# datastax/jvector

Measured on AMD Instinct MI355X. Metric: QPS@recall10>=0.95 (10Mx768); distances/sec as % HBM roofline, higher is better.
Workload: dtype f32

## Files before the change

jvector_amd/csrc/k_gsearch_ubr.hip:

```cpp
#include "jv_device.h"
#include "jv_internal.h"

#define GS_WAVE_SCOPE_BARRIER 1
#define GS_UNIFORM_SHFL 1
#include "gs_wave_hip.h"

#include "gs_body.h"

namespace jv {

static_assert(VSF_L2 == 0 && VSF_DOT == 1 && VSF_COS == 2, "gs_body.h hard-codes the kernel vsf numbering");

template <int VSF, int CH16, bool PROF>
__global__ __launch_bounds__(64) __attribute__((amdgpu_waves_per_eu(2, 2))) void graph_search_ubr_kernel(GsParams p)
{
    extern __shared__ __attribute__((aligned(16))) char gs_lds[];
    gs_worker<VSF, CH16, true, PROF, false, false, true>(p, (int)blockIdx.x, gs_lds);
}

template <int VSF, int CH16, bool PROF>
__global__ __launch_bounds__(64) __attribute__((amdgpu_waves_per_eu(2, 2))) void graph_search_ubrc_kernel(GsParams p)
{
    extern __shared__ __attribute__((aligned(16))) char gs_lds[];
    gs_worker<VSF, CH16, false, PROF, false, true, true>(p, (int)blockIdx.x, gs_lds);
}

constexpr int UBR_QB = 8;

__device__ __forceinline__ int32_t ubr_sortable(float f)
{
    const int32_t b = __builtin_bit_cast(int32_t, f);
    return b ^ ((b >> 31) & 0x7fffffff);
}
__device__ __forceinline__ float ubr_unsortable(int32_t s) { return __builtin_bit_cast(float, s ^ ((s >> 31) & 0x7fffffff)); }

__device__ __forceinline__ void ubr_wave_minmax(float &a, float &b)
{
#define JV_MM_STEP(CTRL)                                      \
    "v_min_f32_dpp %0, %0, %0 " CTRL "\n"                     \
    "v_max_f32_dpp %1, %1, %1 " CTRL "\n"                     \
    "s_nop 0\n"
    asm volatile("s_nop 1\n" JV_MM_STEP("row_shr:1 row_mask:0xf bank_mask:0xf") JV_MM_STEP("row_shr:2 row_mask:0xf bank_mask:0xf")
                     JV_MM_STEP("row_shr:4 row_mask:0xf bank_mask:0xf") JV_MM_STEP("row_shr:8 row_mask:0xf bank_mask:0xf")
                         JV_MM_STEP("row_bcast:15 row_mask:0xa bank_mask:0xf") JV_MM_STEP("row_bcast:31 row_mask:0xc bank_mask:0xf")
                 : "+v"(a), "+v"(b));
#undef JV_MM_STEP
}

template <int VSF>
__global__ __launch_bounds__(256) void ubr_table_kernel(const float *__restrict__ codebooks, const float *__restrict__ cq, int Q, int M,
                                                        uint32_t *__restrict__ tab, float *__restrict__ meta)
{
    extern __shared__ __attribute__((aligned(16))) char ubr_lds[];
    const int D = 8 * M;
    float *qs = reinterpret_cast<float *>(ubr_lds);
    float *lo = qs + UBR_QB * D;
    float *hi = lo + UBR_QB * M;
    float *qS = hi + UBR_QB * M;
    int *qbad = reinterpret_cast<int *>(qS + UBR_QB);
    const int tid = (int)threadIdx.x, lane = tid & 63, wave = tid >> 6;
    const int q0 = (int)blockIdx.x * UBR_QB;
    const int nq = min(UBR_QB, Q - q0);
    for (int i = tid; i < UBR_QB * D / 4; i += 256) {
        const int j = i / (D / 4);
        gs_f4 v = {0.0f, 0.0f, 0.0f, 0.0f};
        if (j < nq) v = reinterpret_cast<const gs_f4 *>(cq + (int64_t)(q0 + j) * D)[i - j * (D / 4)];
        reinterpret_cast<gs_f4 *>(qs)[i] = v;
    }
    if (tid < UBR_QB) qbad[tid] = 0;
    __syncthreads();
    const int H = M / 2, per_wave = H / 4;
    float lo_acc[UBR_QB], hi_acc[UBR_QB];
    uint32_t amax[UBR_QB];
#pragma unroll
    for (int j = 0; j < UBR_QB; ++j) {
        lo_acc[j] = 0.0f;
        hi_acc[j] = 0.0f;
        amax[j] = 0u;
    }
    for (int rr = 0; rr < per_wave; ++rr) {
        const int r = wave * per_wave + rr;
#pragma unroll
        for (int half = 0; half < 2; ++half) {
            const int m = r + half * H;
            gs_f4 c0[4], c1[4];
#pragma unroll
            for (int k = 0; k < 4; ++k) {
                const gs_f4 *cp = reinterpret_cast<const gs_f4 *>(codebooks + ((int64_t)m * 256 + lane + 64 * k) * 8);
                c0[k] = cp[0];
                c1[k] = cp[1];
            }
            const int slot = 2 * rr + half;
#pragma unroll
            for (int j = 0; j < UBR_QB; ++j) {
                const float *q = qs + j * D + m * 8;
                float e4[4];
#pragma unroll
                for (int k = 0; k < 4; ++k) e4[k] = gs_lut_entry_pk<VSF>(c0[k], c1[k], q);
                float fmn = __builtin_fminf(__builtin_fminf(e4[0], e4[1]), __builtin_fminf(e4[2], e4[3]));
                float fmx = __builtin_fmaxf(__builtin_fmaxf(e4[0], e4[1]), __builtin_fmaxf(e4[2], e4[3]));
                uint32_t a = amax[j];
#pragma unroll
                for (int k = 0; k < 4; ++k) {
                    const uint32_t b = __builtin_bit_cast(uint32_t, e4[k]) & 0x7fffffffu;
                    a = b > a ? b : a;
                }
                amax[j] = a;
                ubr_wave_minmax(fmn, fmx);
                const float wmn = __builtin_bit_cast(float, __builtin_amdgcn_readlane(__builtin_bit_cast(int, fmn), 63));
                const float wmx = __builtin_bit_cast(float, __builtin_amdgcn_readlane(__builtin_bit_cast(int, fmx), 63));
                lo_acc[j] = lane == slot ? wmn : lo_acc[j];
                hi_acc[j] = lane == slot ? wmx : hi_acc[j];
            }
        }
    }
#pragma unroll
    for (int j = 0; j < UBR_QB; ++j) {
        if (lane < 2 * per_wave) {
            const int m = wave * per_wave + (lane >> 1) + (lane & 1) * H;
            lo[j * M + m] = lo_acc[j];
            hi[j * M + m] = hi_acc[j];
        }
        if (__ballot(amax[j] >= 0x7f800000u ? 1 : 0) != 0 && lane == 0) qbad[j] = 1;
    }
    __syncthreads();
    if (tid < UBR_QB) {
        const int j = tid;
        float range = 0.0f;
        for (int m = 0; m < M; ++m) {
            const float r = hi[j * M + m] - lo[j * M + m];
            if (r > range) range = r;
        }
        float S = range / 255.0f;
        if (!(S > 1e-30f)) S = 1e-30f;
        float sum_lo = 0.0f, sum_abs = 0.0f, max_abs = 0.0f;
        for (int m = 0; m < M; ++m) {
            const float l = lo[j * M + m], h = hi[j * M + m];
            sum_lo += l;
            const float amn = l < 0.0f ? -l : l, amx = h < 0.0f ? -h : h;
            const float a = amn > amx ? amn : amx;
            sum_abs += a + 256.0f * S;
            if (a > max_abs) max_abs = a;
        }
        const bool ok = qbad[j] == 0 && (sum_abs - sum_abs == 0.0f) && S * 1e6f >= max_abs;
        qS[j] = S;
        if (!ok) qbad[j] = 1;
        if (j < nq) {
            float *mq = meta + (int64_t)(q0 + j) * 4;
            mq[0] = (VSF == VSF_L2) ? sum_lo - 4e-5f * sum_abs : sum_lo + 4e-5f * sum_abs;
            mq[1] = S;
            mq[2] = ok ? 1.0f : 0.0f;
            mq[3] = 0.0f;
        }
    }
    __syncthreads();
    for (int rr = 0; rr < per_wave; ++rr) {
        const int r = wave * per_wave + rr;
        gs_f4 c0[2][4], c1[2][4];
#pragma unroll
        for (int half = 0; half < 2; ++half) {
#pragma unroll
            for (int k = 0; k < 4; ++k) {
                const gs_f4 *cp = reinterpret_cast<const gs_f4 *>(codebooks + ((int64_t)(r + half * H) * 256 + lane + 64 * k) * 8);
                c0[half][k] = cp[0];
                c1[half][k] = cp[1];
            }
        }
        for (int j = 0; j < nq; ++j) {
            const float S = qS[j], inv = 1.0f / S;
            uint32_t b[2][4];
#pragma unroll
            for (int half = 0; half < 2; ++half) {
                const int m = r + half * H;
                const float l = lo[j * M + m];
                const float *q = qs + j * D + m * 8;
                float e4[4];
#pragma unroll
                for (int k = 0; k < 4; ++k) e4[k] = gs_lut_entry_pk<VSF>(c0[half][k], c1[half][k], q);
#pragma unroll
                for (int k = 0; k < 4; ++k) {
                    const float e = e4[k];
                    int bb = (VSF == VSF_L2) ? (int)((e - l) * inv - 0x1p-10f) : (int)((e - l) * inv + 0x1p-10f);
                    bb = bb < 0 ? 0 : (bb > 255 ? 255 : bb);
                    b[half][k] = (uint32_t)bb;
                }
            }
            gs_u2 out;
            out.x = b[0][0] | (b[0][1] << 8) | (b[1][0] << 16) | (b[1][1] << 24);
            out.y = b[0][2] | (b[0][3] << 8) | (b[1][2] << 16) | (b[1][3] << 24);
            if (qbad[j]) out = gs_u2{0u, 0u};
            const int k0 = 2 * r;
            uint32_t *dst = tab + (int64_t)(q0 + j) * M * 64 + ((int64_t)(k0 / 4) * 64 + lane) * 4 + (k0 % 4);
            *reinterpret_cast<gs_u2 *>(dst) = out;
        }
    }
}

size_t ubr_table_lds_bytes(int M) { return sizeof(float) * ((size_t)UBR_QB * 8 * M + 2 * (size_t)UBR_QB * M + UBR_QB) + sizeof(int) * UBR_QB; }

bool graph_search_ubr_supported(int M, int ) { return M == 96; }

int launch_ubr_tables(hipStream_t s, int vsf, const float *codebooks, const float *cq, int Q, int M, uint32_t *tab, float *meta)
{
    if (Q == 0) return JV_OK;
    if (M % 8 != 0) {
        set_error("ubr tables: M a multiple of 8 (M = %d)", M);
        return JV_ERR_INVALID;
    }
    const size_t lds = ubr_table_lds_bytes(M);
    dim3 grid((unsigned)((Q + UBR_QB - 1) / UBR_QB)), block(256);
    if (vsf == VSF_L2) {
        JV_HIP_CHECK(hipFuncSetAttribute((const void *)ubr_table_kernel<VSF_L2>, hipFuncAttributeMaxDynamicSharedMemorySize, (int)lds));
        hipLaunchKernelGGL(ubr_table_kernel<VSF_L2>, grid, block, lds, s, codebooks, cq, Q, M, tab, meta);
    } else if (vsf == VSF_DOT) {
        JV_HIP_CHECK(hipFuncSetAttribute((const void *)ubr_table_kernel<VSF_DOT>, hipFuncAttributeMaxDynamicSharedMemorySize, (int)lds));
        hipLaunchKernelGGL(ubr_table_kernel<VSF_DOT>, grid, block, lds, s, codebooks, cq, Q, M, tab, meta);
    } else {
        JV_HIP_CHECK(hipFuncSetAttribute((const void *)ubr_table_kernel<VSF_COS>, hipFuncAttributeMaxDynamicSharedMemorySize, (int)lds));
        hipLaunchKernelGGL(ubr_table_kernel<VSF_COS>, grid, block, lds, s, codebooks, cq, Q, M, tab, meta);
    }
    JV_HIP_CHECK(hipGetLastError());
    return JV_OK;
}

int launch_graph_search_ubr(hipStream_t s, int vsf, const GsParams &p, int workers, size_t lds)
{
    if (p.Q == 0) return JV_OK;
    if (!p.pair || p.session || p.generic || !graph_search_ubr_supported(p.M, vsf) || !p.ubr_tab || !p.ubr_meta) {
        set_error("graph search kernel: the register-table bound form serves the pair-lane kernels at M = 96");
        return JV_ERR_INVALID;
    }
    dim3 grid(workers), block(64);
#define JV_UBR(VSFV)                                                                                             \
    do {                                                                                                         \
        if (p.pair == 2) {                              \
            hipLaunchKernelGGL((graph_search_ubrc_kernel<VSFV, 6, false>), grid, block, lds, s, p);               \
        } else if (p.prof) hipLaunchKernelGGL((graph_search_ubr_kernel<VSFV, 6, true>), grid, block, lds, s, p);  \
        else hipLaunchKernelGGL((graph_search_ubr_kernel<VSFV, 6, false>), grid, block, lds, s, p);              \
    } while (0)
    if (vsf == VSF_L2) JV_UBR(VSF_L2);
    else if (vsf == VSF_DOT) JV_UBR(VSF_DOT);
    else JV_UBR(VSF_COS);
#undef JV_UBR
    JV_HIP_CHECK(hipGetLastError());
    return JV_OK;
}

}
```

Baseline: 2.515 million.

## Rewrite UBR table kernel with paired-query packed math and permlane reductions

Moves the per-query quantized LUT table builder into its own file and restructures it. Queries are interleaved in pairs in LDS so packed f32 instructions compute two queries' LUT entries at once. Per-subspace min/max is reduced across queries with permlane32/16 swaps plus row DPP rather than a full wave reduction per query. Subspaces are assigned round-robin to waves, and the NaN/Inf check becomes an fma-by-zero accumulator. The aim is to cut ALU and cross-lane reduction cost in table construction, at the price of hand-written inline asm and a new M<=256 limit.

```diff
diff --git a/jvector_amd/csrc/k_gsearch_ubr.hip b/jvector_amd/csrc/k_gsearch_ubr.hip
--- a/jvector_amd/csrc/k_gsearch_ubr.hip
+++ b/jvector_amd/csrc/k_gsearch_ubr.hip
@@ -25,203 +25,7 @@
     gs_worker<VSF, CH16, false, PROF, false, true, true>(p, (int)blockIdx.x, gs_lds);
 }
 
-constexpr int UBR_QB = 8;
-
-__device__ __forceinline__ int32_t ubr_sortable(float f)
-{
-    const int32_t b = __builtin_bit_cast(int32_t, f);
-    return b ^ ((b >> 31) & 0x7fffffff);
-}
-__device__ __forceinline__ float ubr_unsortable(int32_t s) { return __builtin_bit_cast(float, s ^ ((s >> 31) & 0x7fffffff)); }
-
-__device__ __forceinline__ void ubr_wave_minmax(float &a, float &b)
-{
-#define JV_MM_STEP(CTRL)                                      \
-    "v_min_f32_dpp %0, %0, %0 " CTRL "\n"                     \
-    "v_max_f32_dpp %1, %1, %1 " CTRL "\n"                     \
-    "s_nop 0\n"
-    asm volatile("s_nop 1\n" JV_MM_STEP("row_shr:1 row_mask:0xf bank_mask:0xf") JV_MM_STEP("row_shr:2 row_mask:0xf bank_mask:0xf")
-                     JV_MM_STEP("row_shr:4 row_mask:0xf bank_mask:0xf") JV_MM_STEP("row_shr:8 row_mask:0xf bank_mask:0xf")
-                         JV_MM_STEP("row_bcast:15 row_mask:0xa bank_mask:0xf") JV_MM_STEP("row_bcast:31 row_mask:0xc bank_mask:0xf")
-                 : "+v"(a), "+v"(b));
-#undef JV_MM_STEP
-}
-
-template <int VSF>
-__global__ __launch_bounds__(256) void ubr_table_kernel(const float *__restrict__ codebooks, const float *__restrict__ cq, int Q, int M,
-                                                        uint32_t *__restrict__ tab, float *__restrict__ meta)
-{
-    extern __shared__ __attribute__((aligned(16))) char ubr_lds[];
-    const int D = 8 * M;
-    float *qs = reinterpret_cast<float *>(ubr_lds);
-    float *lo = qs + UBR_QB * D;
-    float *hi = lo + UBR_QB * M;
-    float *qS = hi + UBR_QB * M;
-    int *qbad = reinterpret_cast<int *>(qS + UBR_QB);
-    const int tid = (int)threadIdx.x, lane = tid & 63, wave = tid >> 6;
-    const int q0 = (int)blockIdx.x * UBR_QB;
-    const int nq = min(UBR_QB, Q - q0);
-    for (int i = tid; i < UBR_QB * D / 4; i += 256) {
-        const int j = i / (D / 4);
-        gs_f4 v = {0.0f, 0.0f, 0.0f, 0.0f};
-        if (j < nq) v = reinterpret_cast<const gs_f4 *>(cq + (int64_t)(q0 + j) * D)[i - j * (D / 4)];
-        reinterpret_cast<gs_f4 *>(qs)[i] = v;
-    }
-    if (tid < UBR_QB) qbad[tid] = 0;
-    __syncthreads();
-    const int H = M / 2, per_wave = H / 4;
-    float lo_acc[UBR_QB], hi_acc[UBR_QB];
-    uint32_t amax[UBR_QB];
-#pragma unroll
-    for (int j = 0; j < UBR_QB; ++j) {
-        lo_acc[j] = 0.0f;
-        hi_acc[j] = 0.0f;
-        amax[j] = 0u;
-    }
-    for (int rr = 0; rr < per_wave; ++rr) {
-        const int r = wave * per_wave + rr;
-#pragma unroll
-        for (int half = 0; half < 2; ++half) {
-            const int m = r + half * H;
-            gs_f4 c0[4], c1[4];
-#pragma unroll
-            for (int k = 0; k < 4; ++k) {
-                const gs_f4 *cp = reinterpret_cast<const gs_f4 *>(codebooks + ((int64_t)m * 256 + lane + 64 * k) * 8);
-                c0[k] = cp[0];
-                c1[k] = cp[1];
-            }
-            const int slot = 2 * rr + half;
-#pragma unroll
-            for (int j = 0; j < UBR_QB; ++j) {
-                const float *q = qs + j * D + m * 8;
-                float e4[4];
-#pragma unroll
-                for (int k = 0; k < 4; ++k) e4[k] = gs_lut_entry_pk<VSF>(c0[k], c1[k], q);
-                float fmn = __builtin_fminf(__builtin_fminf(e4[0], e4[1]), __builtin_fminf(e4[2], e4[3]));
-                float fmx = __builtin_fmaxf(__builtin_fmaxf(e4[0], e4[1]), __builtin_fmaxf(e4[2], e4[3]));
-                uint32_t a = amax[j];
-#pragma unroll
-                for (int k = 0; k < 4; ++k) {
-                    const uint32_t b = __builtin_bit_cast(uint32_t, e4[k]) & 0x7fffffffu;
-                    a = b > a ? b : a;
-                }
-                amax[j] = a;
-                ubr_wave_minmax(fmn, fmx);
-                const float wmn = __builtin_bit_cast(float, __builtin_amdgcn_readlane(__builtin_bit_cast(int, fmn), 63));
-                const float wmx = __builtin_bit_cast(float, __builtin_amdgcn_readlane(__builtin_bit_cast(int, fmx), 63));
-                lo_acc[j] = lane == slot ? wmn : lo_acc[j];
-                hi_acc[j] = lane == slot ? wmx : hi_acc[j];
-            }
-        }
-    }
-#pragma unroll
-    for (int j = 0; j < UBR_QB; ++j) {
-        if (lane < 2 * per_wave) {
-            const int m = wave * per_wave + (lane >> 1) + (lane & 1) * H;
-            lo[j * M + m] = lo_acc[j];
-            hi[j * M + m] = hi_acc[j];
-        }
-        if (__ballot(amax[j] >= 0x7f800000u ? 1 : 0) != 0 && lane == 0) qbad[j] = 1;
-    }
-    __syncthreads();
-    if (tid < UBR_QB) {
-        const int j = tid;
-        float range = 0.0f;
-        for (int m = 0; m < M; ++m) {
-            const float r = hi[j * M + m] - lo[j * M + m];
-            if (r > range) range = r;
-        }
-        float S = range / 255.0f;
-        if (!(S > 1e-30f)) S = 1e-30f;
-        float sum_lo = 0.0f, sum_abs = 0.0f, max_abs = 0.0f;
-        for (int m = 0; m < M; ++m) {
-            const float l = lo[j * M + m], h = hi[j * M + m];
-            sum_lo += l;
-            const float amn = l < 0.0f ? -l : l, amx = h < 0.0f ? -h : h;
-            const float a = amn > amx ? amn : amx;
-            sum_abs += a + 256.0f * S;
-            if (a > max_abs) max_abs = a;
-        }
-        const bool ok = qbad[j] == 0 && (sum_abs - sum_abs == 0.0f) && S * 1e6f >= max_abs;
-        qS[j] = S;
-        if (!ok) qbad[j] = 1;
-        if (j < nq) {
-            float *mq = meta + (int64_t)(q0 + j) * 4;
-            mq[0] = (VSF == VSF_L2) ? sum_lo - 4e-5f * sum_abs : sum_lo + 4e-5f * sum_abs;
-            mq[1] = S;
-            mq[2] = ok ? 1.0f : 0.0f;
-            mq[3] = 0.0f;
-        }
-    }
-    __syncthreads();
-    for (int rr = 0; rr < per_wave; ++rr) {
-        const int r = wave * per_wave + rr;
-        gs_f4 c0[2][4], c1[2][4];
-#pragma unroll
-        for (int half = 0; half < 2; ++half) {
-#pragma unroll
-            for (int k = 0; k < 4; ++k) {
-                const gs_f4 *cp = reinterpret_cast<const gs_f4 *>(codebooks + ((int64_t)(r + half * H) * 256 + lane + 64 * k) * 8);
-                c0[half][k] = cp[0];
-                c1[half][k] = cp[1];
-            }
-        }
-        for (int j = 0; j < nq; ++j) {
-            const float S = qS[j], inv = 1.0f / S;
-            uint32_t b[2][4];
-#pragma unroll
-            for (int half = 0; half < 2; ++half) {
-                const int m = r + half * H;
-                const float l = lo[j * M + m];
-                const float *q = qs + j * D + m * 8;
-                float e4[4];
-#pragma unroll
-                for (int k = 0; k < 4; ++k) e4[k] = gs_lut_entry_pk<VSF>(c0[half][k], c1[half][k], q);
-#pragma unroll
-                for (int k = 0; k < 4; ++k) {
-                    const float e = e4[k];
-                    int bb = (VSF == VSF_L2) ? (int)((e - l) * inv - 0x1p-10f) : (int)((e - l) * inv + 0x1p-10f);
-                    bb = bb < 0 ? 0 : (bb > 255 ? 255 : bb);
-                    b[half][k] = (uint32_t)bb;
-                }
-            }
-            gs_u2 out;
-            out.x = b[0][0] | (b[0][1] << 8) | (b[1][0] << 16) | (b[1][1] << 24);
-            out.y = b[0][2] | (b[0][3] << 8) | (b[1][2] << 16) | (b[1][3] << 24);
-            if (qbad[j]) out = gs_u2{0u, 0u};
-            const int k0 = 2 * r;
-            uint32_t *dst = tab + (int64_t)(q0 + j) * M * 64 + ((int64_t)(k0 / 4) * 64 + lane) * 4 + (k0 % 4);
-            *reinterpret_cast<gs_u2 *>(dst) = out;
-        }
-    }
-}
-
-size_t ubr_table_lds_bytes(int M) { return sizeof(float) * ((size_t)UBR_QB * 8 * M + 2 * (size_t)UBR_QB * M + UBR_QB) + sizeof(int) * UBR_QB; }
-
 bool graph_search_ubr_supported(int M, int ) { return M == 96; }
-
-int launch_ubr_tables(hipStream_t s, int vsf, const float *codebooks, const float *cq, int Q, int M, uint32_t *tab, float *meta)
-{
-    if (Q == 0) return JV_OK;
-    if (M % 8 != 0) {
-        set_error("ubr tables: M a multiple of 8 (M = %d)", M);
-        return JV_ERR_INVALID;
-    }
-    const size_t lds = ubr_table_lds_bytes(M);
-    dim3 grid((unsigned)((Q + UBR_QB - 1) / UBR_QB)), block(256);
-    if (vsf == VSF_L2) {
-        JV_HIP_CHECK(hipFuncSetAttribute((const void *)ubr_table_kernel<VSF_L2>, hipFuncAttributeMaxDynamicSharedMemorySize, (int)lds));
-        hipLaunchKernelGGL(ubr_table_kernel<VSF_L2>, grid, block, lds, s, codebooks, cq, Q, M, tab, meta);
-    } else if (vsf == VSF_DOT) {
-        JV_HIP_CHECK(hipFuncSetAttribute((const void *)ubr_table_kernel<VSF_DOT>, hipFuncAttributeMaxDynamicSharedMemorySize, (int)lds));
-        hipLaunchKernelGGL(ubr_table_kernel<VSF_DOT>, grid, block, lds, s, codebooks, cq, Q, M, tab, meta);
-    } else {
-        JV_HIP_CHECK(hipFuncSetAttribute((const void *)ubr_table_kernel<VSF_COS>, hipFuncAttributeMaxDynamicSharedMemorySize, (int)lds));
-        hipLaunchKernelGGL(ubr_table_kernel<VSF_COS>, grid, block, lds, s, codebooks, cq, Q, M, tab, meta);
-    }
-    JV_HIP_CHECK(hipGetLastError());
-    return JV_OK;
-}
 
 int launch_graph_search_ubr(hipStream_t s, int vsf, const GsParams &p, int workers, size_t lds)
 {
diff --git a/jvector_amd/csrc/k_ubr_table.hip b/jvector_amd/csrc/k_ubr_table.hip
--- /dev/null
+++ b/jvector_amd/csrc/k_ubr_table.hip
@@ -0,0 +1,287 @@
+#include "jv_device.h"
+#include "jv_internal.h"
+
+namespace jv {
+
+namespace {
+
+constexpr int UBR_QB = 8;
+constexpr int UBR_QP = UBR_QB / 2;
+constexpr int UBR_WAVES = 4;
+constexpr int UBR_MAX_M = 256;
+
+typedef float ubr_f2 __attribute__((ext_vector_type(2)));
+typedef float ubr_f4 __attribute__((ext_vector_type(4)));
+typedef uint32_t ubr_u2 __attribute__((ext_vector_type(2)));
+
+template <int VSF>
+__device__ __forceinline__ ubr_f2 ubr_entry2(const ubr_f4 c0, const ubr_f4 c1, const ubr_f2 *q)
+{
+    const ubr_f2 a = {c0.x, c0.y}, b = {c0.z, c0.w}, c = {c1.x, c1.y}, d = {c1.z, c1.w};
+    ubr_f2 ent, t;
+    if (VSF == VSF_L2) {
+#define JV_UBR_STEP(SEL, C, Q) "v_pk_add_f32 %1, " C ", " Q " " SEL " neg_lo:[0,1] neg_hi:[0,1]\n" "v_pk_mul_f32 %1, %1, %1\n" "v_pk_add_f32 %0, %0, %1\n"
+        asm("v_pk_add_f32 %1, %2, %6 op_sel_hi:[0,1] neg_lo:[0,1] neg_hi:[0,1]\n"
+            "v_pk_mul_f32 %1, %1, %1\n"
+            "v_pk_add_f32 %0, %1, 0 op_sel_hi:[1,0]\n"
+            JV_UBR_STEP("op_sel:[1,0]", "%2", "%7") JV_UBR_STEP("op_sel_hi:[0,1]", "%3", "%8") JV_UBR_STEP("op_sel:[1,0]", "%3", "%9")
+            JV_UBR_STEP("op_sel_hi:[0,1]", "%4", "%10") JV_UBR_STEP("op_sel:[1,0]", "%4", "%11")
+            JV_UBR_STEP("op_sel_hi:[0,1]", "%5", "%12") JV_UBR_STEP("op_sel:[1,0]", "%5", "%13")
+            : "=&v"(ent), "=&v"(t)
+            : "v"(a), "v"(b), "v"(c), "v"(d), "v"(q[0]), "v"(q[1]), "v"(q[2]), "v"(q[3]), "v"(q[4]), "v"(q[5]), "v"(q[6]), "v"(q[7]));
+#undef JV_UBR_STEP
+    } else {
+#define JV_UBR_STEP(SEL, C, Q) "v_pk_mul_f32 %1, " C ", " Q " " SEL "\n" "v_pk_add_f32 %0, %0, %1\n"
+        asm("v_pk_mul_f32 %1, %2, %6 op_sel_hi:[0,1]\n"
+            "v_pk_add_f32 %0, %1, 0 op_sel_hi:[1,0]\n"
+            JV_UBR_STEP("op_sel:[1,0]", "%2", "%7") JV_UBR_STEP("op_sel_hi:[0,1]", "%3", "%8") JV_UBR_STEP("op_sel:[1,0]", "%3", "%9")
+            JV_UBR_STEP("op_sel_hi:[0,1]", "%4", "%10") JV_UBR_STEP("op_sel:[1,0]", "%4", "%11")
+            JV_UBR_STEP("op_sel_hi:[0,1]", "%5", "%12") JV_UBR_STEP("op_sel:[1,0]", "%5", "%13")
+            : "=&v"(ent), "=&v"(t)
+            : "v"(a), "v"(b), "v"(c), "v"(d), "v"(q[0]), "v"(q[1]), "v"(q[2]), "v"(q[3]), "v"(q[4]), "v"(q[5]), "v"(q[6]), "v"(q[7]));
+#undef JV_UBR_STEP
+    }
+    return ent;
+}
+
+__device__ __forceinline__ float ubr_min(float a, float b)
+{
+    float r;
+    asm("v_min_f32 %0, %1, %2" : "=v"(r) : "v"(a), "v"(b));
+    return r;
+}
+__device__ __forceinline__ float ubr_max(float a, float b)
+{
+    float r;
+    asm("v_max_f32 %0, %1, %2" : "=v"(r) : "v"(a), "v"(b));
+    return r;
+}
+__device__ __forceinline__ void ubr_minmax4(float e0, float e1, float e2, float e3, float &mn, float &mx)
+{
+    asm("v_min_f32 %0, %2, %3\n"
+        "v_max_f32 %1, %2, %3\n"
+        "v_min3_f32 %0, %0, %4, %5\n"
+        "v_max3_f32 %1, %1, %4, %5"
+        : "=&v"(mn), "=&v"(mx) : "v"(e0), "v"(e1), "v"(e2), "v"(e3));
+}
+
+__device__ __forceinline__ float ubr_swap_fold(float a, float b, bool lanes32, bool is_min)
+{
+    const uint32_t ua = __builtin_bit_cast(uint32_t, a), ub = __builtin_bit_cast(uint32_t, b);
+    float x, y;
+    if (lanes32) {
+        const auto r = __builtin_amdgcn_permlane32_swap(ua, ub, false, false);
+        x = __builtin_bit_cast(float, (uint32_t)r[0]);
+        y = __builtin_bit_cast(float, (uint32_t)r[1]);
+    } else {
+        const auto r = __builtin_amdgcn_permlane16_swap(ua, ub, false, false);
+        x = __builtin_bit_cast(float, (uint32_t)r[0]);
+        y = __builtin_bit_cast(float, (uint32_t)r[1]);
+    }
+    return is_min ? ubr_min(x, y) : ubr_max(x, y);
+}
+
+__device__ __forceinline__ int ubr_fold_query(int rho) { return ((rho & 1) << 1) | (rho >> 1); }
+__device__ __forceinline__ void ubr_fold_extremes(float (&mn)[UBR_QB], float (&mx)[UBR_QB])
+{
+    float a[4], b[4];
+#pragma unroll
+    for (int i = 0; i < 4; ++i) {
+        a[i] = ubr_swap_fold(mn[2 * i], mn[2 * i + 1], true, true);
+        b[i] = ubr_swap_fold(mx[2 * i], mx[2 * i + 1], true, false);
+    }
+#pragma unroll
+    for (int k = 0; k < 2; ++k) {
+        mn[k] = ubr_swap_fold(a[2 * k], a[2 * k + 1], false, true);
+        mx[k] = ubr_swap_fold(b[2 * k], b[2 * k + 1], false, false);
+    }
+#define JV_UBR_ROW_STEP(CTRL)                                      \
+    "v_min_f32_dpp %0, %0, %0 " CTRL " row_mask:0xf bank_mask:0xf\n" \
+    "v_min_f32_dpp %1, %1, %1 " CTRL " row_mask:0xf bank_mask:0xf\n" \
+    "v_max_f32_dpp %2, %2, %2 " CTRL " row_mask:0xf bank_mask:0xf\n" \
+    "v_max_f32_dpp %3, %3, %3 " CTRL " row_mask:0xf bank_mask:0xf\n"
+    asm volatile("s_nop 1\n" JV_UBR_ROW_STEP("row_shr:1") JV_UBR_ROW_STEP("row_shr:2") JV_UBR_ROW_STEP("row_shr:4") JV_UBR_ROW_STEP("row_shr:8")
+                 : "+v"(mn[0]), "+v"(mn[1]), "+v"(mx[0]), "+v"(mx[1]));
+#undef JV_UBR_ROW_STEP
+}
+
+template <int VSF>
+__global__ __launch_bounds__(64 * UBR_WAVES) __attribute__((amdgpu_waves_per_eu(4))) void ubr_table_kernel(const float *__restrict__ codebooks, const float *__restrict__ cq, int Q,
+                                                                    int M, uint32_t *__restrict__ tab, float *__restrict__ meta)
+{
+    extern __shared__ __attribute__((aligned(16))) char ubr_lds[];
+    const int D = 8 * M, H = M / 2;
+    ubr_f2 *qp = reinterpret_cast<ubr_f2 *>(ubr_lds);
+    float *lo = reinterpret_cast<float *>(qp + UBR_QP * D);
+    float *hi = lo + M * UBR_QB;
+    float *qinv = hi + M * UBR_QB;
+    int *qbad = reinterpret_cast<int *>(qinv + UBR_QB);
+    const int tid = (int)threadIdx.x, lane = tid & 63, wave = tid >> 6;
+    const int q0 = (int)blockIdx.x * UBR_QB;
+    const int nq = min(UBR_QB, Q - q0);
+    for (int i = tid; i < UBR_QP * D / 2; i += 64 * UBR_WAVES) {
+        const int p = i / (D / 2), d2 = i - p * (D / 2);
+        ubr_f2 a = {0.0f, 0.0f}, b = {0.0f, 0.0f};
+        if (2 * p < nq) a = reinterpret_cast<const ubr_f2 *>(cq + (int64_t)(q0 + 2 * p) * D)[d2];
+        if (2 * p + 1 < nq) b = reinterpret_cast<const ubr_f2 *>(cq + (int64_t)(q0 + 2 * p + 1) * D)[d2];
+        reinterpret_cast<ubr_f4 *>(qp)[i] = ubr_f4{a.x, b.x, a.y, b.y};
+    }
+    if (tid < UBR_QB) qbad[tid] = 0;
+    __syncthreads();
+
+    ubr_f2 nonfinite[UBR_QP];
+#pragma unroll
+    for (int p = 0; p < UBR_QP; ++p) nonfinite[p] = ubr_f2{0.0f, 0.0f};
+    for (int m = wave; m < M; m += UBR_WAVES) {
+        ubr_f4 c0[4], c1[4];
+#pragma unroll
+        for (int k = 0; k < 4; ++k) {
+            const ubr_f4 *cp = reinterpret_cast<const ubr_f4 *>(codebooks + ((int64_t)m * 256 + lane + 64 * k) * 8);
+            c0[k] = cp[0];
+            c1[k] = cp[1];
+        }
+        float mn[UBR_QB], mx[UBR_QB];
+#pragma unroll
+        for (int p = 0; p < UBR_QP; ++p) {
+            ubr_f2 q[8];
+#pragma unroll
+            for (int t = 0; t < 8; ++t) q[t] = qp[p * D + m * 8 + t];
+            ubr_f2 e[4];
+#pragma unroll
+            for (int k = 0; k < 4; ++k) {
+                e[k] = ubr_entry2<VSF>(c0[k], c1[k], q);
+                nonfinite[p] = __builtin_elementwise_fma(e[k], ubr_f2{0.0f, 0.0f}, nonfinite[p]);
+            }
+            ubr_minmax4(e[0].x, e[1].x, e[2].x, e[3].x, mn[2 * p], mx[2 * p]);
+            ubr_minmax4(e[0].y, e[1].y, e[2].y, e[3].y, mn[2 * p + 1], mx[2 * p + 1]);
+        }
+        ubr_fold_extremes(mn, mx);
+        if ((lane & 15) == 15) {
+            const int j = ubr_fold_query(lane >> 4);
+#pragma unroll
+            for (int k = 0; k < 2; ++k) {
+                lo[m * UBR_QB + 4 * k + j] = mn[k];
+                hi[m * UBR_QB + 4 * k + j] = mx[k];
+            }
+        }
+    }
+#pragma unroll
+    for (int p = 0; p < UBR_QP; ++p) {
+        const bool ba = __ballot(nonfinite[p].x != nonfinite[p].x ? 1 : 0) != 0;
+        const bool bb = __ballot(nonfinite[p].y != nonfinite[p].y ? 1 : 0) != 0;
+        if (lane == 0 && ba) qbad[2 * p] = 1;
+        if (lane == 0 && bb) qbad[2 * p + 1] = 1;
+    }
+    __syncthreads();
+
+    if (tid < UBR_QB) {
+        const int j = tid;
+        float range = 0.0f;
+        for (int m = 0; m < M; ++m) {
+            const float r = hi[m * UBR_QB + j] - lo[m * UBR_QB + j];
+            if (r > range) range = r;
+        }
+        float S = range / 255.0f;
+        if (!(S > 1e-30f)) S = 1e-30f;
+        float sum_lo = 0.0f, sum_abs = 0.0f, max_abs = 0.0f;
+        for (int m = 0; m < M; ++m) {
+            const float l = lo[m * UBR_QB + j], h = hi[m * UBR_QB + j];
+            sum_lo += l;
+            const float amn = l < 0.0f ? -l : l, amx = h < 0.0f ? -h : h;
+            const float a = amn > amx ? amn : amx;
+            sum_abs += a + 256.0f * S;
+            if (a > max_abs) max_abs = a;
+        }
+        const bool ok = qbad[j] == 0 && (sum_abs - sum_abs == 0.0f) && S * 1e6f >= max_abs;
+        qinv[j] = 1.0f / S;
+        if (!ok) qbad[j] = 1;
+        if (j < nq) {
+            float *mq = meta + (int64_t)(q0 + j) * 4;
+            mq[0] = (VSF == VSF_L2) ? sum_lo - 4e-5f * sum_abs : sum_lo + 4e-5f * sum_abs;
+            mq[1] = S;
+            mq[2] = ok ? 1.0f : 0.0f;
+            mq[3] = 0.0f;
+        }
+    }
+    __syncthreads();
+
+    const ubr_f2 edge = (VSF == VSF_L2) ? ubr_f2{-0x1p-10f, -0x1p-10f} : ubr_f2{0x1p-10f, 0x1p-10f};
+    for (int r = wave; r < H; r += UBR_WAVES) {
+        uint32_t w[UBR_QB][2];
+#pragma unroll
+        for (int j = 0; j < UBR_QB; ++j) w[j][0] = w[j][1] = 0u;
+#pragma unroll
+        for (int half = 0; half < 2; ++half) {
+            const int m = r + half * H;
+            ubr_f4 c0[4], c1[4];
+#pragma unroll
+            for (int k = 0; k < 4; ++k) {
+                const ubr_f4 *cp = reinterpret_cast<const ubr_f4 *>(codebooks + ((int64_t)m * 256 + lane + 64 * k) * 8);
+                c0[k] = cp[0];
+                c1[k] = cp[1];
+            }
+#pragma unroll
+            for (int p = 0; p < UBR_QP; ++p) {
+                if (2 * p >= nq) continue;
+                const ubr_f2 inv = *reinterpret_cast<const ubr_f2 *>(qinv + 2 * p);
+                const ubr_f2 l = *reinterpret_cast<const ubr_f2 *>(lo + m * UBR_QB + 2 * p);
+                ubr_f2 q[8];
+#pragma unroll
+                for (int t = 0; t < 8; ++t) q[t] = qp[p * D + m * 8 + t];
+#pragma unroll
+                for (int k = 0; k < 4; ++k) {
+                    const ubr_f2 x = (ubr_entry2<VSF>(c0[k], c1[k], q) - l) * inv + edge;
+                    int ba = (int)x.x, bb = (int)x.y;
+                    ba = ba < 0 ? 0 : (ba > 255 ? 255 : ba);
+                    bb = bb < 0 ? 0 : (bb > 255 ? 255 : bb);
+                    w[2 * p][k >> 1] |= (uint32_t)ba << (8 * (k & 1) + 16 * half);
+                    w[2 * p + 1][k >> 1] |= (uint32_t)bb << (8 * (k & 1) + 16 * half);
+                }
+            }
+        }
+        const int k0 = 2 * r;
+        const int64_t off = ((int64_t)(k0 / 4) * 64 + lane) * 4 + (k0 % 4);
+#pragma unroll
+        for (int j = 0; j < UBR_QB; ++j) {
+            if (j >= nq) continue;
+            ubr_u2 out = {w[j][0], w[j][1]};
+            if (qbad[j]) out = ubr_u2{0u, 0u};
+            *reinterpret_cast<ubr_u2 *>(tab + (int64_t)(q0 + j) * M * 64 + off) = out;
+        }
+    }
+}
+
+size_t ubr_table_lds_bytes(int M)
+{
+    return sizeof(float) * ((size_t)UBR_QB * 8 * M + 2 * (size_t)UBR_QB * M + UBR_QB) + sizeof(int) * UBR_QB;
+}
+
+}
+
+int launch_ubr_tables(hipStream_t s, int vsf, const float *codebooks, const float *cq, int Q, int M, uint32_t *tab, float *meta)
+{
+    if (Q == 0) return JV_OK;
+    if (M <= 0 || M % 8 != 0) {
+        set_error("ubr tables: M a multiple of 8 (M = %d)", M);
+        return JV_ERR_INVALID;
+    }
+    if (M > UBR_MAX_M) {
+        set_error("ubr tables: M = %d (at most %d subspaces)", M, UBR_MAX_M);
+        return JV_ERR_UNSUPPORTED;
+    }
+    const size_t lds = ubr_table_lds_bytes(M);
+    dim3 grid((unsigned)((Q + UBR_QB - 1) / UBR_QB)), block(64 * UBR_WAVES);
+#define JV_UBR_TABLES(VSFV)                                                                                                             \
+    do {                                                                                                                                \
+        JV_HIP_CHECK(hipFuncSetAttribute((const void *)ubr_table_kernel<VSFV>, hipFuncAttributeMaxDynamicSharedMemorySize, (int)lds)); \
+        hipLaunchKernelGGL(ubr_table_kernel<VSFV>, grid, block, lds, s, codebooks, cq, Q, M, tab, meta);                                \
+    } while (0)
+    if (vsf == VSF_L2) JV_UBR_TABLES(VSF_L2);
+    else if (vsf == VSF_DOT) JV_UBR_TABLES(VSF_DOT);
+    else JV_UBR_TABLES(VSF_COS);
+#undef JV_UBR_TABLES
+    JV_HIP_CHECK(hipGetLastError());
+    return JV_OK;
+}
+
+}
```

New measurement: 2.553 million, median of 6. +1.5%, better.
